# ekinakyurek/Long-Term-Recurrent-Convolutional-NN

Measured on AMD Instinct MI355X. Metric: training images/sec (VGG16+LSTM, COCO, batch 256) at 1/2/4/8 MI355X, higher is better.
Workload: dtype bf16

## Files before the change

long-term-recurrent-convolutional-nn_amd/_lib.py:

```python
import ctypes as C
import os
import subprocess

HERE = os.path.dirname(os.path.abspath(__file__))
CSRC = os.path.join(HERE, "csrc")
LIB_PATH = os.environ.get("LRCN_HIP_LIB") or os.path.join(CSRC, "liblrcn_hip.so")
HEADER = os.path.normpath(os.path.join(HERE, "..", "include", "lrcn.h"))
SAMPLE_HEADER = os.path.normpath(os.path.join(HERE, "..", "include", "lrcn_sample.h"))
SCORE_HEADER = os.path.normpath(os.path.join(HERE, "..", "include", "lrcn_score.h"))
NUCLEUS_HEADER = os.path.normpath(os.path.join(HERE, "..", "include", "lrcn_nucleus.h"))
NBEST_HEADER = os.path.normpath(os.path.join(HERE, "..", "include", "lrcn_nbest.h"))
DIVERSE_HEADER = os.path.normpath(os.path.join(HERE, "..", "include", "lrcn_diverse.h"))
ACTIVITY_HEADER = os.path.normpath(os.path.join(HERE, "..", "include", "lrcn_activity.h"))
ACT_DROPOUT_HEADER = os.path.normpath(os.path.join(HERE, "..", "include", "lrcn_act_dropout.h"))
VARLEN_HEADER = os.path.normpath(os.path.join(HERE, "..", "include", "lrcn_varlen.h"))
CLIP_HEADER = os.path.normpath(os.path.join(HERE, "..", "include", "lrcn_clip.h"))
WEIGHTED_HEADER = os.path.normpath(os.path.join(HERE, "..", "include", "lrcn_weighted.h"))
SCHED_HEADER = os.path.normpath(os.path.join(HERE, "..", "include", "lrcn_sched.h"))
GEMM_DEBUG_HEADER = os.path.normpath(os.path.join(HERE, "..", "include", "lrcn_gemm_debug.h"))
CONV_DEBUG_HEADER = os.path.normpath(os.path.join(HERE, "..", "include", "lrcn_conv_debug.h"))

LRCN_F32, LRCN_BF16, LRCN_FP8 = 0, 1, 2
LRCN_ABI_VERSION = 5
LRCN_OPT_FUSED_UPDATE, LRCN_OPT_DETERMINISTIC, LRCN_OPT_CONV_CHUNK_BYTES = 1, 2, 3
SEGMENTS = ("update", "rec_fwd", "rec_bwd", "embed_gather", "embed_grad", "preprocess", "upload")
EOS, BOS, UNK = 0, 1, 2
CNNOUT = 4096
MAX_T = 28


class LrcnError(RuntimeError):
    pass


class Config(C.Structure):
    _fields_ = [("device", C.c_int), ("E", C.c_int), ("H1", C.c_int), ("H2", C.c_int), ("V", C.c_int),
                ("max_B", C.c_int), ("max_T", C.c_int), ("lstm_dtype", C.c_int), ("vgg_dtype", C.c_int),
                ("max_images", C.c_int), ("n_layers", C.c_int)]


class ActConfig(C.Structure):
    _fields_ = [("device", C.c_int), ("F", C.c_int), ("H", C.c_int), ("C", C.c_int), ("max_B", C.c_int), ("max_T", C.c_int),
                ("dtype", C.c_int), ("deterministic", C.c_int)]


class ActDropout(C.Structure):
    _fields_ = [("p_in", C.c_float), ("p_out", C.c_float), ("seed", C.c_uint64), ("mask_in", C.c_void_p), ("mask_out", C.c_void_p)]


class GemmDebug(C.Structure):
    _fields_ = [("dtype", C.c_int), ("A", C.c_void_p), ("B", C.c_void_p), ("C", C.c_void_p), ("bias", C.c_void_p),
                ("lda", C.c_int64), ("ldb", C.c_int64), ("ldc", C.c_int64), ("M", C.c_int), ("N", C.c_int), ("K", C.c_int),
                ("c_f32", C.c_int), ("beta", C.c_int), ("relu", C.c_int), ("c_is_zero", C.c_int), ("deterministic", C.c_int),
                ("free_cus", C.c_int), ("bg_cus", C.c_int), ("wg_cap", C.c_int)]


class ConvGemmDebug(C.Structure):
    _fields_ = [("dtype", C.c_int), ("x", C.c_void_p), ("w", C.c_void_p), ("bias", C.c_void_p), ("y", C.c_void_p), ("ldc", C.c_int64),
                ("N", C.c_int), ("H", C.c_int), ("W", C.c_int), ("Cin", C.c_int), ("Cout", C.c_int), ("relu", C.c_int), ("pool", C.c_int),
                ("wg_cap", C.c_int)]


class Dropout(C.Structure):
    _fields_ = [("pdrop", C.c_float), ("seed", C.c_uint64), ("mask1", C.c_void_p), ("mask2", C.c_void_p)]


class Sched(C.Structure):
    _fields_ = [("eps", C.c_float), ("temperature", C.c_float), ("seed", C.c_uint64), ("row0", C.c_int64)]


P9 = C.c_void_p * 9
P4 = C.c_void_p * 4
P13 = C.c_void_p * 13

SIGNATURES = {
    "lrcn_create": (C.c_int, [C.POINTER(Config), C.POINTER(C.c_void_p)]),
    "lrcn_destroy": (None, [C.c_void_p]),
# ... 163 lines not shown
CLIP_SIGNATURES = {
    "lrcn_grad_sumsq": (C.c_int, [C.c_void_p, C.c_void_p, C.c_int64, C.c_int, C.c_void_p]),
    "lrcn_grad_sumsq_model": (C.c_int, [C.c_void_p, P9, C.c_int, C.c_void_p]),
    "lrcn_clip_slots": (C.c_int, [C.c_void_p, C.POINTER(C.c_void_p)]),
    "lrcn_clip_set": (C.c_int, [C.c_void_p, C.c_int, C.c_float, C.c_void_p]),
    "lrcn_adam_update_clipped": (C.c_int, [C.c_void_p, P9, P9, P9, P9, C.c_int, C.c_float, C.c_float, C.c_float, C.c_float]),
    "lrcn_adam_update_group_clipped": (C.c_int, [C.c_void_p, P9, P9, P9, P9, C.c_int, C.c_int, C.c_float, C.c_float, C.c_float, C.c_float,
                                                 C.c_void_p]),
    "lrcn_adam_update_flat_clipped": (C.c_int, [C.c_void_p, C.c_void_p, C.c_void_p, C.c_void_p, C.c_void_p, C.c_int64, C.c_int, C.c_float,
                                                C.c_float, C.c_float, C.c_float, C.c_void_p]),
    "lrcn_train_step_clip": (C.c_int, [C.c_void_p, P9, P9, P9, P9, C.c_void_p, C.c_void_p, C.c_int, C.c_int, C.c_int, C.POINTER(Dropout),
                                       C.c_int, C.c_float, C.c_float, C.c_float, C.c_float, C.c_float, C.POINTER(C.c_double)]),
    "lrcn_train_step_var_clip": (C.c_int, [C.c_void_p, P9, P9, P9, P9, C.c_void_p, C.c_void_p, C.POINTER(C.c_int32), C.c_int, C.c_int,
                                           C.c_int64, C.POINTER(Dropout), C.c_int, C.c_float, C.c_float, C.c_float, C.c_float, C.c_float,
                                           C.POINTER(C.c_double)]),
    "lrcn_clip_stats": (C.c_int, [C.c_void_p, C.POINTER(ClipStats)]),
}

GEMM_DEBUG_SIGNATURES = {
    "lrcn_debug_gemm": (C.c_int, [C.c_void_p, C.POINTER(GemmDebug)]),
    "lrcn_debug_conv_gemm": (C.c_int, [C.c_void_p, C.POINTER(ConvGemmDebug)]),
}

CONV_DEBUG_SIGNATURES = {
    "lrcn_debug_conv11": (C.c_int, [C.c_void_p, C.c_void_p, C.c_int, C.c_int, C.c_int, C.POINTER(C.c_float), C.c_void_p, C.c_void_p, C.c_void_p]),
    "lrcn_debug_fp8_cast": (C.c_int, [C.c_void_p, C.c_int, C.c_void_p, C.c_int64, C.c_float, C.c_void_p]),
    "lrcn_debug_amax": (C.c_int, [C.c_void_p, C.c_void_p, C.c_int64, C.c_void_p]),
    "lrcn_debug_conv64_f8": (C.c_int, [C.c_void_p, C.c_void_p, C.c_int, C.c_int, C.c_int, C.c_void_p, C.c_void_p, C.c_int, C.c_float, C.c_void_p]),
    "lrcn_debug_fp8_scales": (C.c_int, [C.c_void_p, C.POINTER(C.c_float)]),
}


def build(force=False):
    srcs = [os.path.join(CSRC, f) for f in os.listdir(CSRC) if f.endswith((".hip", ".h"))] + [HEADER, SAMPLE_HEADER, NUCLEUS_HEADER, SCORE_HEADER, NBEST_HEADER, DIVERSE_HEADER,
                                                                                                   ACTIVITY_HEADER, ACT_DROPOUT_HEADER, VARLEN_HEADER, CLIP_HEADER, WEIGHTED_HEADER, SCHED_HEADER, GEMM_DEBUG_HEADER, CONV_DEBUG_HEADER]
    stale = force or not os.path.exists(LIB_PATH) or os.path.getmtime(LIB_PATH) < max(os.path.getmtime(s) for s in srcs)
    if stale:
        subprocess.check_call(["make", "-s", "-j4", "-C", CSRC, "-f", os.path.join(CSRC, "Makefile")])
    return LIB_PATH


_LIB = None


def lib():
    global _LIB
    if _LIB is None:
        if not os.path.exists(LIB_PATH):
            raise LrcnError("%s is missing: run `python -c 'import __graft_entry__ as g; g.build()'` "
                            "(there is no CPU fallback)" % LIB_PATH)
        import torch
        L = C.CDLL(LIB_PATH)
        for name, (res, args) in list(SIGNATURES.items()) + list(SAMPLE_SIGNATURES.items()) + list(NUCLEUS_SIGNATURES.items()) + list(SCORE_SIGNATURES.items()) + list(NBEST_SIGNATURES.items()) + list(DIVERSE_SIGNATURES.items()) + \
                list(ACTIVITY_SIGNATURES.items()) + list(ACT_DROPOUT_SIGNATURES.items()) + list(VARLEN_SIGNATURES.items()) + list(CLIP_SIGNATURES.items()) + list(WEIGHTED_SIGNATURES.items()) + list(SCHED_SIGNATURES.items()) + \
                list(GEMM_DEBUG_SIGNATURES.items()) + list(CONV_DEBUG_SIGNATURES.items()):
            fn = getattr(L, name)
            fn.restype = res
            fn.argtypes = args
        if L.lrcn_abi_version() != LRCN_ABI_VERSION:
            raise LrcnError("%s implements ABI revision %d, this binding was written against %d (lrcn_config's layout differs)"
                            % (LIB_PATH, L.lrcn_abi_version(), LRCN_ABI_VERSION))
        _LIB = L
    return _LIB


def check(ctx_handle, rc):
    if rc != 0:
        msg = lib().lrcn_last_error(ctx_handle)
        raise LrcnError("liblrcn_hip error %d: %s" % (rc, msg.decode() if msg else "?"))
```

long-term-recurrent-convolutional-nn_amd/csrc/ctx.h:

```cpp
#pragma once
#include <utility>

#include "comm.h"
#include "host.h"
#include "../../include/lrcn_sched.h"

namespace lrcn_impl {

struct VggLayer {
    void *w = nullptr;
    void *w_fused = nullptr;
    float *b = nullptr;
    int Cin = 0, Cout = 0, S = 0, pool = 0;
    void *w8 = nullptr;
    float *sw = nullptr, *escale = nullptr, *ebias = nullptr;
};
constexpr int kFp8First = 3;

}

struct lrcn_ctx {
    lrcn_config cfg{};
    hipStream_t stream = nullptr;
    std::string err;
// ... 80 lines not shown
    int vgg_wg_cap = 0;
    bool vgg_loaded = false;
    bool vgg_fp8 = false, fp8_ready = false;
    float *amax_dev = nullptr;
    float act_scale[13] = {};
    lrcn_impl::VggLayer conv[13];
    void *fc6w = nullptr, *fc7w = nullptr;
    float *fc6b = nullptr, *fc7b = nullptr;
    void *actA = nullptr, *actB = nullptr, *im2col = nullptr, *f6 = nullptr, *img16 = nullptr;
    float *featsRM = nullptr;
    bool prof = false;
    std::vector<std::pair<hipEvent_t, hipEvent_t>> prof_ev;
    size_t prof_used = 0;
    double prof_ms = 0.0;
    int64_t prof_launches = 0;
    int prof_level = 0;
    struct SegProf {
        std::vector<std::pair<hipEvent_t, hipEvent_t>> ev;
        size_t used = 0;
        double ms = 0.0, bytes = 0.0;
        int64_t n = 0;
    } seg[LRCN_SEG_COUNT];
    std::string vgg_routes;
    float *avg_img = nullptr;
    bool avg_on = false;
    void *img_meta = nullptr;
    int img_meta_cap = 0;
    float *pre_f32 = nullptr;
    hipStream_t wg_stream = nullptr;
    bool wg_stream_owned = true;
    hipEvent_t wg_fork[4] = {}, wg_done = nullptr;
    hipEvent_t xc_fork = nullptr, xc_done = nullptr;
    void *wg_ws = nullptr;
    void *pin = nullptr;
    size_t pin_bytes = 0;
    unsigned long long *stamps = nullptr;
    int64_t stamps_n = 0;
    int *tile_ctr = nullptr;
    static constexpr int kStage = 3;
    hipStream_t copy_stream = nullptr;
    uint8_t *stage[kStage] = {};
    hipEvent_t up_done[kStage] = {}, rd_done[kStage] = {};
    bool stage_full[kStage] = {};
    bool stage_read[kStage] = {};
    int stage_next = 0;
    LrcnComm *comm = nullptr;
// ... 18 lines not shown
        auto &sp = c->seg[seg];
        if (sp.used == sp.ev.size()) {
            std::pair<hipEvent_t, hipEvent_t> e;
            if (hipEventCreate(&e.first) != hipSuccess || hipEventCreate(&e.second) != hipSuccess) return;
            sp.ev.push_back(e);
        }
        ev = &sp.ev[sp.used++];
        sp.bytes += bytes;
        sp.n += 1;
        (void)hipEventRecord(ev->first, st);
    }
    ~SegScope() {
        if (ev) (void)hipEventRecord(ev->second, st);
    }
};

inline hipStream_t stream_or_ctx(lrcn_ctx *c, void *stream) { return stream ? reinterpret_cast<hipStream_t>(stream) : c->stream; }
inline void ctx_sizes(const lrcn_ctx *c, int64_t sz[9]) { lrcn_param_sizes_n(c->nl, c->E, c->H1, c->H2, c->V, sz); }
constexpr int kGradGroup[LRCN_GRAD_GROUPS][2] = {{7, 8}, {2, 3}, {4, 5}, {0, 1}, {6, 6}};

int gemm(lrcn_ctx *c, int dtype, const void *A, int64_t lda, const void *B, int64_t ldb, void *C, int64_t ldc, int M, int N, int K,
         const float *bias, bool c_f32, bool beta = false, bool relu = false, bool c_is_zero = false, bool on_wg_stream = false);

#define GEMM(...)                     \
    do {                              \
        int _r = gemm(__VA_ARGS__);   \
        if (_r) return _r;            \
    } while (0)

void set_create_error(const char *msg);
int step_internal(lrcn_ctx *c, const float *const p[9], int B, const DropSpec &d2, bool h_ready = false);
struct LossCall {
    const float *const *p = nullptr;
    const float *feats = nullptr;
    const int32_t *tokens = nullptr;
    int T = 0, B = 0, norm_B = 1;
    int64_t norm_tokens = 0;
    const lrcn_dropout *drop = nullptr;
    float *const *grads = nullptr;
    const int32_t *lens = nullptr;
    const float *row_w = nullptr;
    const lrcn_sched *ss = nullptr;
    int32_t *fed_out = nullptr;
    float *logits_out = nullptr;
    enum Form { PLAIN, VAR, WEIGHTED, SCHED } form = PLAIN;
};
// ... 20 lines not shown
```

long-term-recurrent-convolutional-nn_amd/csrc/gemm.h:

```cpp
#pragma once
#include <hip/hip_runtime.h>
#include <stdint.h>

enum { GEMM_A_PLAIN = 0, GEMM_A_CONV3 = 1 };
enum { GEMM_OUT_PLAIN = 0, GEMM_OUT_CONV = 1, GEMM_OUT_POOL = 2, GEMM_OUT_LSTM_FWD = 3, GEMM_OUT_LSTM_BWD = 4, GEMM_OUT_SMAX_TOPK = 5,
       GEMM_OUT_SMAX_GUMBEL = 6, GEMM_OUT_SMAX_PICK = 7 };

enum { SMAX_KC = 6, SMAX_REC = 16 };
enum { SMAX_MAX_NREC = 256 };
struct SmaxEpi {
    float *part;
    int nrec;
    float temp;
    uint32_t key0, key1;
    int current, S;
    const int32_t *tgt;
};

struct LstmEpi {
    int H;
    int64_t ld_a, ld_h;
    const float *Gx;
    const float *c_prev;
    const int *c_prev_idx;
// ... 46 lines not shown
};

constexpr int kBgMinRows = 256, kBgMaxRows = 512;
inline bool bg_row_window(int rows) { return rows >= kBgMinRows && rows <= kBgMaxRows; }

hipError_t launch_gemm(hipStream_t stream, const GemmArgs &g);
hipError_t launch_gemm_nt(hipStream_t stream, const GemmArgs &g);

void gemm_debug_note_route(const char *route, int cfg);
const char *gemm_debug_last_route();

bool gemm_glds_eligible(const GemmArgs &g);
hipError_t launch_gemm_glds(hipStream_t stream, const GemmArgs &g);
int64_t gemm_glds_blocks(const GemmArgs &g);

int gemm_8p_config(const GemmArgs &g, int64_t *blocks);
int gemm_8p_splitk(const GemmArgs &g, int64_t *blocks);
hipError_t launch_gemm_8p(hipStream_t stream, const GemmArgs &g, int splitk = 1);
hipError_t launch_splitk_reduce(hipStream_t stream, const GemmArgs &g, int splits);

bool gemm_skinny_eligible(const GemmArgs &g);
hipError_t launch_gemm_skinny(hipStream_t stream, const GemmArgs &g);

bool conv64_eligible(int dtype, int Cin, int Cout, int H, int W);
hipError_t launch_conv64(hipStream_t stream, const void *in, const void *w, const float *bias, void *out, int N, int H, int W, int Cout,
                         int relu, int pool, const void *zero_page, float f8_inv_scale = 0.0f, int wg_cap = 0, unsigned long long *stamps = nullptr);
hipError_t launch_conv64_fused11(hipStream_t stream, const void *img16, const void *w11, const float *b11, const void *w,
                                 const float *bias, void *out, int N, int S, const void *zero_page, int wg_cap = 0, unsigned long long *stamps = nullptr);
hipError_t launch_conv64f(hipStream_t stream, const void *img16, const void *w11, const void *w, const float *bias, void *out, int N, int S,
                          const void *zero_page, int wg_cap = 0, unsigned long long *stamps = nullptr);
```

long-term-recurrent-convolutional-nn_amd/csrc/lrcn_api.hip:

```cpp
#include <algorithm>
#include <cmath>

#include "ctx.h"

static thread_local std::string g_create_err;
using namespace lrcn_impl;

constexpr int kBgWgsPerFreeCu = 4;

int lrcn_impl::gemm(lrcn_ctx *c, int dtype, const void *A, int64_t lda, const void *B, int64_t ldb, void *C, int64_t ldc, int M, int N,
         int K, const float *bias, bool c_f32, bool beta, bool relu, bool c_is_zero, bool on_wg_stream) {
    GemmArgs g{};
    g.dtype = dtype;
    g.A = A;
    g.lda = lda;
    g.B = B;
    g.ldb = ldb;
    g.C = C;
    g.ldc = ldc;
    g.M = M;
    g.N = N;
    g.K = gemm_k(dtype, lda, ldb, K);
    g.bias = bias;
    g.c_f32 = c_f32;
    g.beta = beta;
    g.c_is_zero = c_is_zero;
    g.relu = relu;
    g.a_mode = GEMM_A_PLAIN;
    g.out_mode = GEMM_OUT_PLAIN;
    g.zero_page = c->zero_page;
    g.deterministic = c->opt_det;
    g.ws = on_wg_stream ? c->wg_ws : c->gemm_ws;
    g.ws_bytes = c->gemm_ws_bytes;
    if (!lstm_alone(c)) {
        const int free_cus = std::max(c->ncu - c->vgg_wg_cap, 0);
        if (c->cur_B < kBgMinRows) {
            g.free_cus = free_cus;
        } else {
            g.bg_cus = free_cus;
            if (free_cus >= 8) g.wg_cap = free_cus * kBgWgsPerFreeCu;
        }
    }
    hipError_t e = launch_gemm(on_wg_stream ? c->wg_stream : c->stream, g);
    if (e != hipSuccess) FAIL(c, LRCN_EHIP, "gemm M=%d N=%d K=%d: %s", M, N, K, hipGetErrorString(e));
    if (knob_char("LRCN_TRACE_ROUTES") == '1') {
        fprintf(stderr, "gemm M=%d N=%d K=%d %s-> %s\n", M, N, K, on_wg_stream ? "(wg stream) " : "", gemm_debug_last_route());
    }
    return LRCN_OK;
}

void lrcn_impl::set_create_error(const char *msg) { g_create_err = msg; }

int lrcn_impl::step_internal(lrcn_ctx *c, const float *const p[9], int B, const DropSpec &d2, bool h_ready) {
    const int dt = c->dt, E = c->E, H1 = c->H1, H2 = c->H2, h = c->h, V = c->V, X1 = c->X1;
    hipStream_t st = c->stream;
    const bool two = c->nl == 2;
    if (!two) k_concat_x2(st, dt, c->st_x, c->ldX1, c->xcnn, c->ldh, 1, B, E, h, d2);
    if (!h_ready) k_cast_rows(st, dt, c->st_f32[0], H1, B, H1, c->st_h1, c->ldH1);
    GEMM(c, dt, c->st_x, c->ldX1, c->W1x, c->ldX1, c->st_g, 4 * H1, B, 4 * H1, X1, p[1], true);
    GEMM(c, dt, c->st_h1, c->ldH1, c->W1h, c->ldH1, c->st_g, 4 * H1, B, 4 * H1, H1, nullptr, true, true);
    k_lstm_fwd(st, dt, c->st_g, 4 * H1, c->st_f32[1], B, H1, c->st_a, c->ld4H1, c->st_f32[1], c->st_h1, c->ldH1, c->st_f32[0]);
    if (!two) {
        GEMM(c, dt, c->st_h1, c->ldH1, c->Wod, c->ldH2, c->st_logits, c->ldV, B, V, H2, p[8], true);
// ... 370 lines not shown
        k_mul_f32(st, x_lstm, mask1, (int64_t)B * E, c->st_io);
        xsrc = c->st_io;
    }
    k_transpose(st, dt, 1, xsrc, B, E, B, c->st_x, c->ldX1, 0);
    r = step_internal(c, p, B, d2);
    if (r) return r;
    for (int i = 0; i < ns; ++i) k_transpose_f32(st, c->st_f32[i], Hs[i], B, Hs[i], state[i], B);
    k_transpose_f32(st, c->st_logits, c->ldV, B, V, logits, B);
    KCHK(c, "lrcn_step");
    return LRCN_OK;
}

int lrcn_debug_stamps(lrcn_ctx *c, unsigned long long *host_out, int64_t n) {
    DeviceGuard dg(c);
    if (!c || !host_out || n < 1) return LRCN_EINVAL;
    if (!c->stamps || n > c->stamps_n) FAIL(c, LRCN_ESTATE, "no stamps recorded (LRCN_STAMPS=1 and lrcn_bench_conv first), or n > %lld", (long long)c->stamps_n);
    HIPCHK(c, hipStreamSynchronize(c->stream));
    HIPCHK(c, hipMemcpy(host_out, c->stamps, sizeof(unsigned long long) * (size_t)n, hipMemcpyDeviceToHost));
    return LRCN_OK;
}

const char *lrcn_debug_route(lrcn_ctx *c, int which) {
    if (which == 1) return c ? c->vgg_routes.c_str() : "";
    return gemm_debug_last_route();
}

int lrcn_profile(lrcn_ctx *c, int enable) {
    DeviceGuard dg(c);
    if (!c) return LRCN_EINVAL;
    c->prof = enable != 0;
    c->prof_level = enable;
    c->prof_used = 0;
    c->prof_ms = 0.0;
    c->prof_launches = 0;
    for (auto &sp : c->seg) {
        sp.used = 0;
        sp.ms = sp.bytes = 0.0;
        sp.n = 0;
    }
    return LRCN_OK;
}

int lrcn_profile_segment(lrcn_ctx *c, int segment, double *ms, int64_t *brackets, double *bytes) {
    DeviceGuard dg(c);
    if (!c || !ms || !brackets || !bytes || segment < 0 || segment >= LRCN_SEG_COUNT) return LRCN_EINVAL;
    HIPCHK(c, hipDeviceSynchronize());
// ... 31 lines not shown
```

long-term-recurrent-convolutional-nn_amd/csrc/train.hip:

```cpp
#include <cmath>
#include <cstring>

#include "ctx.h"
#include "../../include/lrcn_varlen.h"
#include "../../include/lrcn_clip.h"
#include "../../include/lrcn_weighted.h"
#include "../../include/lrcn_sched.h"

using namespace lrcn_impl;

namespace {

DropSpec make_drop(const lrcn_dropout *d, int which) {
    DropSpec s{};
    s.which = which;
    if (d) {
        s.p = d->pdrop;
        s.seed = d->seed;
        s.mask = which == 1 ? d->mask1 : d->mask2;
        if (s.mask) s.p = 0.0f;
    }
    return s;
}

// ... 277 lines not shown
    if (c->opt_det && !c->logp_rows) DALLOC(c, c->logp_rows, sizeof(double) * (size_t)c->maxS * c->maxB);
    void *const dlog = bwd ? c->dLog : nullptr;
    double *const rows = c->opt_det ? c->logp_rows : nullptr;
    if (q.row_w) k_softmax_xent_weighted(st, dt, c->Logits, c->ldV, c->tok_tgt, M, V, scale, c->logp, dlog, c->ldV, rows, c->roww_dev, B);
    else (q.lens ? k_softmax_xent_masked : k_softmax_xent)(st, dt, c->Logits, c->ldV, c->tok_tgt, M, V, scale, c->logp, dlog, c->ldV, rows);
    c->last_norm = q.norm_B;
    c->last_S = S;
    c->last_tokens = q.lens ? q.norm_tokens : 0;
    KCHK(c, "forward");
    if (!bwd) return LRCN_OK;

    const int64_t ldM = ld64(M), ldB = ld64(B);
    hipStream_t sw = par ? c->wg_stream : st;
    int nfork = 0;
    auto fork = [&]() -> int {
        if (!par) return LRCN_OK;
        HIPCHK(c, hipEventRecord(c->wg_fork[nfork], st));
        HIPCHK(c, hipStreamWaitEvent(sw, c->wg_fork[nfork], 0));
        ++nfork;
        return LRCN_OK;
    };
    auto weight_grad = [&](const void *dY, int64_t ldY, int NY, const void *x, int64_t ldx, int X, const void *Hprev, int64_t ldHp, int Hp,
                           float *dW, float *db) -> int {
        TrPlan pl{};
        auto tr = [&](const void *src, int64_t ld_src, int R, int C, void *dst, int shift) {
            TrDesc &d = pl.d[pl.n++];
            d.src = src; d.ld_src = ld_src; d.R = R; d.C = C; d.dst = dst; d.ld_dst = ldM; d.shift = shift;
        };
        tr(dY, ldY, M, NY, c->TA, 0);
        tr(x, ldx, M, X, c->TB, 0);
        if (Hprev) tr(Hprev, ldHp, M - B, Hp, boff(c->TB, (int64_t)X * ldM, es), M > B ? B : 0);
        k_transpose_multi(sw, dt, pl);
        const int Xh = X + (Hprev ? Hp : 0);
        GEMM(c, dt, c->TA, ldM, c->TB, ldM, dW, Xh, NY, Xh, M, nullptr, true, false, false, false, par);
        if (db) k_colsum(sw, dt, dY, ldY, M, NY, db, c->opt_det);
        return LRCN_OK;
    };
    auto image_embedding_grad = [&]() -> int {
        k_transpose(sw, dt, 1, c->dxcnn, c->ldh, B, h, c->dxcT, ldB, 0);
        k_cast_rows(sw, dt, q.feats, B, LRCN_CNNOUT, B, c->FT, ldB);
        GEMM(c, dt, c->dxcT, ldB, c->FT, ldB, q.grads[5], LRCN_CNNOUT, h, LRCN_CNNOUT, B, nullptr, true, false, false, false, par);
        HIPCHK(c, hipEventRecord(c->grad_ev[2], sw));
        return LRCN_OK;
    };
    auto backward = [&]() -> int {
        if (int e = fork()) return e;
        if (int e = weight_grad(c->dLog, c->ldV, V, Htop, c->ldH2, H2, nullptr, 0, 0, q.grads[7], q.grads[8])) return e;
        HIPCHK(c, hipEventRecord(c->grad_ev[0], sw));
        GEMM(c, dt, c->dLog, c->ldV, c->WoT, c->ldV, two ? c->dH2all : c->dH1all, H2, M, H2, V, nullptr, true);
        if (two) {
            if (int e = lstm_layer_bwd(c, S, B, H2, c->ld4H2, c->A2, c->C2, c->dH2all, c->W2hT, c->dZ2)) return e;
            if (int e = fork()) return e;
            if (int e = weight_grad(c->dZ2, c->ld4H2, 4 * H2, c->X2, c->ldH2, H2, c->H2all, c->ldH2, H2, q.grads[2], q.grads[3])) return e;
        }
        HIPCHK(c, hipEventRecord(c->grad_ev[1], sw));
        if (two) {
            GEMM(c, dt, c->dZ2, c->ld4H2, c->W2xT, c->ld4H2, c->dX2, c->ldH2, M, H2, 4 * H2, nullptr, false);
// ... 256 lines not shown
```

long-term-recurrent-convolutional-nn_amd/csrc/vgg.hip:

```cpp
#include <algorithm>
#include <cstring>

#include "ctx.h"
#include "../../include/lrcn_conv_debug.h"
#include "../../include/lrcn_gemm_debug.h"

using namespace lrcn_impl;

static const int kVggCout[13] = {64, 64, 128, 128, 256, 256, 256, 512, 512, 512, 512, 512, 512};
static const int kVggPool[13] = {0, 1, 0, 1, 0, 0, 1, 0, 0, 1, 0, 0, 1};

namespace {
int stamps_reserve(lrcn_ctx *c, int64_t need) {
    if (need > c->stamps_n) {
        c->stamps = nullptr;
        DALLOC(c, c->stamps, sizeof(unsigned long long) * (size_t)need);
        c->stamps_n = need;
    }
    return LRCN_OK;
}
bool conv64_enabled() { return !knob_off("LRCN_CONV64"); }
constexpr int kTileCtrStride = 8 + 2 * 512;
hipError_t launch_conv_chunked(hipStream_t st, const GemmArgs &g0, int N, int es, int64_t limit_bytes = 0) {
    const int64_t per_img = (int64_t)g0.H * g0.W * g0.Cin * es;
    int64_t cap = ((limit_bytes > 0 ? limit_bytes : 0xF0000000ll) - (limit_bytes > 0 ? 0 : (int64_t)(g0.W + 1) * g0.Cin * es)) / per_img;
    if (limit_bytes > 0 && cap < 1) cap = 1;
    if (N <= cap || cap < 1) return launch_gemm(st, g0);
    const int nch = (int)((N + cap - 1) / cap), per = (N + nch - 1) / nch;
// ... 385 lines not shown
    g.N = d->N;
    g.K = d->K;
    g.bias = d->bias;
    g.c_f32 = d->c_f32 != 0;
    g.beta = d->beta != 0;
    g.c_is_zero = d->c_is_zero != 0;
    g.relu = d->relu != 0;
    g.a_mode = GEMM_A_PLAIN;
    g.out_mode = GEMM_OUT_PLAIN;
    g.zero_page = c->zero_page;
    g.deterministic = d->deterministic != 0;
    g.ws = c->gemm_ws;
    g.ws_bytes = c->gemm_ws_bytes;
    g.free_cus = d->free_cus;
    g.bg_cus = d->bg_cus;
    g.wg_cap = d->wg_cap;
    const hipError_t e = launch_gemm(c->stream, g);
    if (e != hipSuccess)
        FAIL(c, e == hipErrorInvalidValue ? LRCN_EINVAL : LRCN_EHIP, "debug_gemm M=%d N=%d K=%d: %s", d->M, d->N, d->K, hipGetErrorString(e));
    HIPCHK(c, hipStreamSynchronize(c->stream));
    return LRCN_OK;
}

int lrcn_debug_conv_gemm(lrcn_ctx *c, const lrcn_conv_gemm_debug *d) {
    DeviceGuard dg(c);
    if (!c || !d) return LRCN_EINVAL;
    if (d->dtype != LRCN_F32 && d->dtype != LRCN_BF16) FAIL(c, LRCN_EINVAL, "debug_conv_gemm: dtype %d is neither f32 nor bf16", d->dtype);
    if (d->N < 1 || d->H < 2 || d->W < 2 || d->Cin < 1 || d->Cout < 1 || d->ldc < d->Cout || (int64_t)d->N * d->H * d->W > 0x7FFFFFFF ||
        (int64_t)9 * d->Cin > 0x7FFFFFFF)
        FAIL(c, LRCN_EINVAL, "debug_conv_gemm: N=%d H=%d W=%d Cin=%d Cout=%d ldc=%lld", d->N, d->H, d->W, d->Cin, d->Cout, (long long)d->ldc);
    GemmArgs g{};
    g.dtype = d->dtype == LRCN_BF16 ? GEMM_T_BF16 : GEMM_T_F32;
    g.A = d->x;
    g.B = d->w;
    g.ldb = 9 * (int64_t)d->Cin;
    g.C = d->y;
    g.ldc = d->ldc;
    g.M = d->N * d->H * d->W;
    g.N = d->Cout;
    g.K = 9 * d->Cin;
    g.bias = d->bias;
    g.relu = d->relu != 0;
    g.a_mode = GEMM_A_CONV3;
    g.out_mode = d->pool ? GEMM_OUT_POOL : GEMM_OUT_CONV;
    g.H = d->H;
    g.W = d->W;
// ... 452 lines not shown
```

long-term-recurrent-convolutional-nn_amd/lrcn.py:

```python
import ctypes as C

import numpy as np
import torch

from . import _lib
from ._lib import BOS, CNNOUT, EOS, LRCN_BF16, LRCN_F32, LRCN_FP8, UNK, LrcnError

PARAM_NAMES = ("W1", "b1", "W2", "b2", "Wproj", "Wcnn", "Wembed", "Wout", "bout")
VGG_COUT = (64, 64, 128, 128, 256, 256, 256, 512, 512, 512, 512, 512, 512)
VGG_MEAN = (123.68, 116.779, 103.939)


def jl_empty(*dims, device="cuda", dtype=torch.float32):
    t = torch.empty(tuple(reversed(dims)), device=device, dtype=dtype)
    return t.permute(*reversed(range(len(dims))))


def jl_zeros(*dims, device="cuda", dtype=torch.float32):
    t = jl_empty(*dims, device=device, dtype=dtype)
    t.zero_()
    return t


def to_jl(a, device="cuda"):
# ... 787 lines not shown

def debug_route(ctx, which=0):
    r = _lib.lib().lrcn_debug_route(ctx._h, int(which))
    return r.decode() if r else ""


def debug_gemm(ctx, dtype, A, B, Cmat, M, N, K, lda, ldb, ldc, bias=None, c_f32=False, beta=False, relu=False, c_is_zero=False,
               deterministic=False, free_cus=0, bg_cus=0, wg_cap=0):
    def addr(t):
        if t is None:
            return None
        if torch.is_tensor(t):
            if not t.is_cuda:
                raise LrcnError("expected a CUDA (HIP) tensor")
            return C.c_void_p(t.data_ptr())
        return C.c_void_p(int(t))
    g = _lib.GemmDebug(int(dtype), addr(A), addr(B), addr(Cmat), addr(bias), int(lda), int(ldb), int(ldc), int(M), int(N), int(K),
                       int(bool(c_f32)), int(bool(beta)), int(bool(relu)), int(bool(c_is_zero)), int(bool(deterministic)),
                       int(free_cus), int(bg_cus), int(wg_cap))
    ctx._call("lrcn_debug_gemm", C.byref(g))
    return debug_route(ctx, 0)


def debug_conv_gemm(ctx, dtype, x, w, y, N, H, W, Cin, Cout, ldc, bias=None, relu=False, pool=False, wg_cap=0):
    def addr(t):
        if t is None:
            return None
        if torch.is_tensor(t):
            if not t.is_cuda:
                raise LrcnError("expected a CUDA (HIP) tensor")
            return C.c_void_p(t.data_ptr())
        return C.c_void_p(int(t))
    g = _lib.ConvGemmDebug(int(dtype), addr(x), addr(w), addr(bias), addr(y), int(ldc), int(N), int(H), int(W), int(Cin), int(Cout),
                           int(bool(relu)), int(bool(pool)), int(wg_cap))
    ctx._call("lrcn_debug_conv_gemm", C.byref(g))
    return debug_route(ctx, 0)


def synthetic_vgg_weights(seed=1, device="cuda", bias_std=0.0):
    g = torch.Generator(device=device)
    g.manual_seed(seed)
    conv_w, conv_b = [], []
    cin = 3
    for cout in VGG_COUT:
        w = jl_empty(3, 3, cin, cout, device=device)
        w.copy_(torch.randn((3, 3, cin, cout), generator=g, device=device) * float(np.sqrt(2.0 / (9 * cin))))
# ... 11 lines not shown
```

Before: 37640.

## Add transposed-input bf16 GEMM kernel for LSTM weight gradients, skipping explicit transposes

Adds a dedicated MFMA GEMM kernel that computes dY^T·[x,Hprev] directly from row-major inputs. It uses transposing LDS reads (ds_read_b64_tr_b16), a 4-stage async global-to-LDS pipeline, and two segments per launch. The LSTM weight-gradient path uses it by default for bf16, which removes the transpose kernels and the scratch buffers they wrote. It adds a large hand-tuned kernel with tile heuristics. If the kernel is ineligible, the old transpose-plus-GEMM path still runs.

```diff
diff --git a/include/lrcn_gemm_tn_debug.h b/include/lrcn_gemm_tn_debug.h
--- /dev/null
+++ b/include/lrcn_gemm_tn_debug.h
@@ -0,0 +1,28 @@
+#ifndef LRCN_GEMM_TN_DEBUG_H
+#define LRCN_GEMM_TN_DEBUG_H
+
+#include "lrcn.h"
+
+#ifdef __cplusplus
+extern "C" {
+#endif
+
+typedef struct lrcn_gemm_tn_debug {
+    const void *A;
+    const void *B;
+    float *C;
+    int64_t lda, ldb, ldc;
+    int M, NA, NB;
+    int shift;
+    int tile;
+} lrcn_gemm_tn_debug;
+
+int lrcn_debug_gemm_tn(lrcn_ctx *ctx, const lrcn_gemm_tn_debug *g);
+
+int lrcn_debug_set_wgrad_tn(lrcn_ctx *ctx, int on);
+
+#ifdef __cplusplus
+}
+#endif
+
+#endif
diff --git a/long-term-recurrent-convolutional-nn_amd/_lib.py b/long-term-recurrent-convolutional-nn_amd/_lib.py
--- a/long-term-recurrent-convolutional-nn_amd/_lib.py
+++ b/long-term-recurrent-convolutional-nn_amd/_lib.py
@@ -18,6 +18,7 @@
 WEIGHTED_HEADER = os.path.normpath(os.path.join(HERE, "..", "include", "lrcn_weighted.h"))
 SCHED_HEADER = os.path.normpath(os.path.join(HERE, "..", "include", "lrcn_sched.h"))
 GEMM_DEBUG_HEADER = os.path.normpath(os.path.join(HERE, "..", "include", "lrcn_gemm_debug.h"))
+GEMM_TN_DEBUG_HEADER = os.path.normpath(os.path.join(HERE, "..", "include", "lrcn_gemm_tn_debug.h"))
 CONV_DEBUG_HEADER = os.path.normpath(os.path.join(HERE, "..", "include", "lrcn_conv_debug.h"))
 
 LRCN_F32, LRCN_BF16, LRCN_FP8 = 0, 1, 2
@@ -53,6 +54,11 @@
                 ("lda", C.c_int64), ("ldb", C.c_int64), ("ldc", C.c_int64), ("M", C.c_int), ("N", C.c_int), ("K", C.c_int),
                 ("c_f32", C.c_int), ("beta", C.c_int), ("relu", C.c_int), ("c_is_zero", C.c_int), ("deterministic", C.c_int),
                 ("free_cus", C.c_int), ("bg_cus", C.c_int), ("wg_cap", C.c_int)]
+
+
+class GemmTnDebug(C.Structure):
+    _fields_ = [("A", C.c_void_p), ("B", C.c_void_p), ("C", C.c_void_p), ("lda", C.c_int64), ("ldb", C.c_int64), ("ldc", C.c_int64),
+                ("M", C.c_int), ("NA", C.c_int), ("NB", C.c_int), ("shift", C.c_int), ("tile", C.c_int)]
 
 
 class ConvGemmDebug(C.Structure):
@@ -262,6 +268,11 @@
     "lrcn_debug_conv_gemm": (C.c_int, [C.c_void_p, C.POINTER(ConvGemmDebug)]),
 }
 
+GEMM_TN_DEBUG_SIGNATURES = {
+    "lrcn_debug_gemm_tn": (C.c_int, [C.c_void_p, C.POINTER(GemmTnDebug)]),
+    "lrcn_debug_set_wgrad_tn": (C.c_int, [C.c_void_p, C.c_int]),
+}
+
 CONV_DEBUG_SIGNATURES = {
     "lrcn_debug_conv11": (C.c_int, [C.c_void_p, C.c_void_p, C.c_int, C.c_int, C.c_int, C.POINTER(C.c_float), C.c_void_p, C.c_void_p, C.c_void_p]),
     "lrcn_debug_fp8_cast": (C.c_int, [C.c_void_p, C.c_int, C.c_void_p, C.c_int64, C.c_float, C.c_void_p]),
@@ -273,7 +284,7 @@
 
 def build(force=False):
     srcs = [os.path.join(CSRC, f) for f in os.listdir(CSRC) if f.endswith((".hip", ".h"))] + [HEADER, SAMPLE_HEADER, NUCLEUS_HEADER, SCORE_HEADER, NBEST_HEADER, DIVERSE_HEADER,
-                                                                                                   ACTIVITY_HEADER, ACT_DROPOUT_HEADER, VARLEN_HEADER, CLIP_HEADER, WEIGHTED_HEADER, SCHED_HEADER, GEMM_DEBUG_HEADER, CONV_DEBUG_HEADER]
+                                                                                                   ACTIVITY_HEADER, ACT_DROPOUT_HEADER, VARLEN_HEADER, CLIP_HEADER, WEIGHTED_HEADER, SCHED_HEADER, GEMM_DEBUG_HEADER, GEMM_TN_DEBUG_HEADER, CONV_DEBUG_HEADER]
     stale = force or not os.path.exists(LIB_PATH) or os.path.getmtime(LIB_PATH) < max(os.path.getmtime(s) for s in srcs)
     if stale:
         subprocess.check_call(["make", "-s", "-j4", "-C", CSRC, "-f", os.path.join(CSRC, "Makefile")])
@@ -293,7 +304,7 @@
         L = C.CDLL(LIB_PATH)
         for name, (res, args) in list(SIGNATURES.items()) + list(SAMPLE_SIGNATURES.items()) + list(NUCLEUS_SIGNATURES.items()) + list(SCORE_SIGNATURES.items()) + list(NBEST_SIGNATURES.items()) + list(DIVERSE_SIGNATURES.items()) + \
                 list(ACTIVITY_SIGNATURES.items()) + list(ACT_DROPOUT_SIGNATURES.items()) + list(VARLEN_SIGNATURES.items()) + list(CLIP_SIGNATURES.items()) + list(WEIGHTED_SIGNATURES.items()) + list(SCHED_SIGNATURES.items()) + \
-                list(GEMM_DEBUG_SIGNATURES.items()) + list(CONV_DEBUG_SIGNATURES.items()):
+                list(GEMM_DEBUG_SIGNATURES.items()) + list(GEMM_TN_DEBUG_SIGNATURES.items()) + list(CONV_DEBUG_SIGNATURES.items()):
             fn = getattr(L, name)
             fn.restype = res
             fn.argtypes = args
diff --git a/long-term-recurrent-convolutional-nn_amd/csrc/ctx.h b/long-term-recurrent-convolutional-nn_amd/csrc/ctx.h
--- a/long-term-recurrent-convolutional-nn_amd/csrc/ctx.h
+++ b/long-term-recurrent-convolutional-nn_amd/csrc/ctx.h
@@ -126,6 +126,8 @@
         int64_t n = 0;
     } seg[LRCN_SEG_COUNT];
     std::string vgg_routes;
+    bool wgrad_tn = true;
+    std::string wgrad_route;
     float *avg_img = nullptr;
     bool avg_on = false;
     void *img_meta = nullptr;
@@ -190,6 +192,8 @@
 int gemm(lrcn_ctx *c, int dtype, const void *A, int64_t lda, const void *B, int64_t ldb, void *C, int64_t ldc, int M, int N, int K,
          const float *bias, bool c_f32, bool beta = false, bool relu = false, bool c_is_zero = false, bool on_wg_stream = false);
 
+int bg_wg_cap(const lrcn_ctx *c);
+
 #define GEMM(...)                     \
     do {                              \
         int _r = gemm(__VA_ARGS__);   \
diff --git a/long-term-recurrent-convolutional-nn_amd/csrc/gemm.h b/long-term-recurrent-convolutional-nn_amd/csrc/gemm.h
--- a/long-term-recurrent-convolutional-nn_amd/csrc/gemm.h
+++ b/long-term-recurrent-convolutional-nn_amd/csrc/gemm.h
@@ -92,6 +92,31 @@
 bool gemm_skinny_eligible(const GemmArgs &g);
 hipError_t launch_gemm_skinny(hipStream_t stream, const GemmArgs &g);
 
+struct GemmTnSeg {
+    const void *A;
+    int64_t lda;
+    const void *B;
+    int64_t ldb;
+    float *C;
+    int64_t ldc;
+    int M;
+    int NB;
+    int tile0, vec;
+};
+struct GemmTnArgs {
+    int dtype;
+    GemmTnSeg seg[2];
+    int nseg;
+    int M;
+    int NA;
+    int wg_cap;
+    int tile;
+    const void *zero_page;
+    int tiles;
+};
+bool gemm_tn_eligible(const GemmTnArgs &g);
+hipError_t launch_gemm_tn(hipStream_t stream, const GemmTnArgs &g);
+
 bool conv64_eligible(int dtype, int Cin, int Cout, int H, int W);
 hipError_t launch_conv64(hipStream_t stream, const void *in, const void *w, const float *bias, void *out, int N, int H, int W, int Cout,
                          int relu, int pool, const void *zero_page, float f8_inv_scale = 0.0f, int wg_cap = 0, unsigned long long *stamps = nullptr);
diff --git a/long-term-recurrent-convolutional-nn_amd/csrc/gemm_tn.hip b/long-term-recurrent-convolutional-nn_amd/csrc/gemm_tn.hip
--- /dev/null
+++ b/long-term-recurrent-convolutional-nn_amd/csrc/gemm_tn.hip
@@ -0,0 +1,219 @@
+#include <type_traits>
+#include <utility>
+
+#include "common.h"
+#include "gemm.h"
+
+namespace {
+
+typedef __attribute__((address_space(3))) void lds_void;
+typedef const __attribute__((address_space(1))) void glb_void;
+typedef unsigned u32x2 __attribute__((ext_vector_type(2)));
+typedef unsigned u32x4 __attribute__((ext_vector_type(4)));
+
+constexpr int TN_IMG_COLS = 128;
+constexpr int TN_BK = 32;
+constexpr int TN_NBUF = 4;
+constexpr int TN_IPT = 4;
+constexpr int TN_IMG_BYTES = TN_BK * TN_IMG_COLS * 2;
+static_assert((TN_NBUF - 2) * TN_IPT <= 48, "vmcnt is a 6-bit counter");
+
+template <int NWA, int NWB, int FA, int FB> struct TnCfg {
+    static constexpr int TA = NWA * FA * 16, TB = NWB * FB * 16, NW = NWA * NWB, THREADS = NW * 64;
+    static constexpr int NIA = TA / TN_IMG_COLS, NIB = TB / TN_IMG_COLS;
+    static constexpr int STAGE_BYTES = (NIA + NIB) * TN_IMG_BYTES, LDS_BYTES = TN_NBUF * STAGE_BYTES;
+    static_assert(TA % TN_IMG_COLS == 0 && TB % TN_IMG_COLS == 0 && 2 * (NIA + NIB) == NW, "two waves stage one image");
+};
+
+template <int... I, typename F> __device__ __forceinline__ void tn_static_for(std::integer_sequence<int, I...>, F &&f) {
+    (f(std::integral_constant<int, I>{}), ...);
+}
+
+__device__ __forceinline__ int tn_swz(int k) { return ((k & 3) << 2) | ((k >> 2) & 3); }
+__device__ __forceinline__ int tn_off(int k, int ch) { return 256 * k + 16 * (ch ^ tn_swz(k)); }
+
+template <int N> __device__ __forceinline__ void tn_wait_vmcnt() { asm volatile("s_waitcnt vmcnt(%0)" ::"n"(N) : "memory"); }
+template <int N> __device__ __forceinline__ void tn_wait_lgkmcnt() {
+    asm volatile("s_waitcnt lgkmcnt(%0)" ::"n"(N) : "memory");
+    __builtin_amdgcn_sched_barrier(0);
+}
+__device__ __forceinline__ u32x2 tn_read_tr(unsigned addr) {
+    u32x2 r;
+    asm volatile("ds_read_b64_tr_b16 %0, %1" : "=v"(r) : "v"(addr) : "memory");
+    return r;
+}
+__device__ __forceinline__ bf16x8 tn_pack(u32x2 lo, u32x2 hi) { return __builtin_bit_cast(bf16x8, u32x4{lo[0], lo[1], hi[0], hi[1]}); }
+
+template <int NWA, int NWB, int FA, int FB>
+__global__ __launch_bounds__(NWA * NWB * 64) void gemm_tn_kernel(const GemmTnArgs g) {
+    using Cfg = TnCfg<NWA, NWB, FA, FB>;
+    constexpr int TA = Cfg::TA, TB = Cfg::TB, NIA = Cfg::NIA, STAGE_BYTES = Cfg::STAGE_BYTES;
+    extern __shared__ __attribute__((aligned(16))) unsigned char tn_lds[];
+    const int tid = threadIdx.x, lane = tid & 63;
+    const int wave = __builtin_amdgcn_readfirstlane(tid >> 6);
+    const int wa = wave / NWB, wb = wave % NWB;
+    const int grp = lane >> 4, li = lane & 15, q = li >> 2, p = li & 3;
+    const unsigned lds0 = (unsigned)(uintptr_t)(__attribute__((address_space(3))) unsigned char *)tn_lds;
+    unsigned addr_a[FA][2], addr_b[FB][2];
+#pragma unroll
+    for (int r = 0; r < 2; ++r) {
+        const int k = 8 * grp + 4 * r + q;
+#pragma unroll
+        for (int j = 0; j < FA; ++j) {
+            const int col = (wa * FA + j) * 16;
+            addr_a[j][r] = lds0 + (col / TN_IMG_COLS) * TN_IMG_BYTES + tn_off(k, (col % TN_IMG_COLS) / 8 + (p >> 1)) + 8 * (p & 1);
+        }
+#pragma unroll
+        for (int j = 0; j < FB; ++j) {
+            const int col = (wb * FB + j) * 16;
+            addr_b[j][r] = lds0 + (NIA + col / TN_IMG_COLS) * TN_IMG_BYTES + tn_off(k, (col % TN_IMG_COLS) / 8 + (p >> 1)) + 8 * (p & 1);
+        }
+    }
+    const int img = wave >> 1;
+    const bool stage_a = img < NIA;
+    const int img_col = (stage_a ? img : img - NIA) * TN_IMG_COLS;
+    const int pc0 = (wave & 1) * 4;
+    const unsigned char *zp = static_cast<const unsigned char *>(g.zero_page) + li * 16;
+
+    for (int tile = blockIdx.x; tile < g.tiles; tile += gridDim.x) {
+        const GemmTnSeg s = g.seg[(g.nseg > 1 && tile >= g.seg[1].tile0) ? 1 : 0];
+        const int tb_n = (s.NB + TB - 1) / TB;
+        const int t = tile - s.tile0, a0 = (t / tb_n) * TA, b0 = (t % tb_n) * TB;
+        const int M = s.M, nk = (M + TN_BK - 1) / TN_BK;
+        const bf16_t *P = static_cast<const bf16_t *>(stage_a ? s.A : s.B);
+        const int ld = (int)(stage_a ? s.lda : s.ldb), ncols = stage_a ? g.NA : s.NB, c0 = (stage_a ? a0 : b0) + img_col;
+        int src_off[TN_IPT], src_row[TN_IPT];
+#pragma unroll
+        for (int i = 0; i < TN_IPT; ++i) {
+            const int row = 4 * (pc0 + i) + grp, col = c0 + 8 * (li ^ tn_swz(row));
+            src_row[i] = row;
+            src_off[i] = col < ncols ? row * ld + col : -1;
+        }
+        auto stage = [&](int kt, int slot, bool live) {
+            unsigned char *dst = tn_lds + slot * STAGE_BYTES + img * TN_IMG_BYTES + pc0 * 1024;
+#pragma unroll
+            for (int i = 0; i < TN_IPT; ++i) {
+                const bool ok = live && src_off[i] >= 0 && kt * TN_BK + src_row[i] < M;
+                const void *src = ok ? static_cast<const void *>(P + ((int64_t)kt * TN_BK * ld + src_off[i])) : static_cast<const void *>(zp);
+                __builtin_amdgcn_global_load_lds((glb_void *)src, (lds_void *)(dst + i * 1024), 16, 0, 0);
+            }
+        };
+
+        f32x4 acc[FB][FA];
+#pragma unroll
+        for (int jb = 0; jb < FB; ++jb)
+#pragma unroll
+            for (int ja = 0; ja < FA; ++ja) acc[jb][ja] = f32x4{0.f, 0.f, 0.f, 0.f};
+
+#pragma unroll
+        for (int t0 = 0; t0 < TN_NBUF - 1; ++t0) stage(t0, t0, t0 < nk);
+        for (int kt = 0; kt < nk; ++kt) {
+            tn_wait_vmcnt<(TN_NBUF - 2) * TN_IPT>();
+            __builtin_amdgcn_s_barrier();
+            const int nxt = kt + TN_NBUF - 1;
+            stage(nxt, nxt % TN_NBUF, nxt < nk);
+            const unsigned cur = (unsigned)(kt % TN_NBUF) * STAGE_BYTES;
+            u32x2 rb[FB][2], ra[FA][2];
+#pragma unroll
+            for (int j = 0; j < FB; ++j) {
+                rb[j][0] = tn_read_tr(addr_b[j][0] + cur);
+                rb[j][1] = tn_read_tr(addr_b[j][1] + cur);
+            }
+#pragma unroll
+            for (int j = 0; j < FA; ++j) {
+                ra[j][0] = tn_read_tr(addr_a[j][0] + cur);
+                ra[j][1] = tn_read_tr(addr_a[j][1] + cur);
+            }
+            tn_static_for(std::make_integer_sequence<int, FA>{}, [&](auto col) {
+                constexpr int ja = decltype(col)::value;
+                tn_wait_lgkmcnt<2 * (FA - 1 - ja)>();
+#pragma unroll
+                for (int jb = 0; jb < FB; ++jb)
+                    acc[jb][ja] = __builtin_amdgcn_mfma_f32_16x16x32_bf16(tn_pack(rb[jb][0], rb[jb][1]), tn_pack(ra[ja][0], ra[ja][1]), acc[jb][ja], 0, 0, 0);
+            });
+            __builtin_amdgcn_sched_barrier(0);
+        }
+        tn_wait_vmcnt<0>();
+
+        float *C = s.C;
+#pragma unroll
+        for (int ja = 0; ja < FA; ++ja) {
+            const int row = a0 + 16 * (FA * wa + ja) + li;
+            if (row >= g.NA) continue;
+            float *crow = C + (int64_t)row * s.ldc;
+#pragma unroll
+            for (int jb = 0; jb < FB; ++jb) {
+                const int col = b0 + 16 * (FB * wb + jb) + 4 * grp;
+                const f32x4 v = acc[jb][ja];
+                if (col + 4 <= s.NB && s.vec == 4) {
+                    *reinterpret_cast<f32x4 *>(crow + col) = v;
+                } else if (col + 4 <= s.NB && s.vec == 2) {
+                    *reinterpret_cast<float2 *>(crow + col) = make_float2(v[0], v[1]);
+                    *reinterpret_cast<float2 *>(crow + col + 2) = make_float2(v[2], v[3]);
+                } else {
+#pragma unroll
+                    for (int e = 0; e < 4; ++e)
+                        if (col + e < s.NB) crow[col + e] = v[e];
+                }
+            }
+        }
+        tn_wait_vmcnt<0>();
+        __syncthreads();
+    }
+}
+
+bool seg_ok(const GemmTnSeg &s, int NA, int M) {
+    if (!s.A || !s.B || !s.C || s.M < 0 || s.M > M || s.NB < 1) return false;
+    if (((uintptr_t)s.A & 15) || ((uintptr_t)s.B & 15) || ((uintptr_t)s.C & 3)) return false;
+    if ((s.lda & 7) || (s.ldb & 7) || s.lda < NA || s.ldb < s.NB || s.ldc < s.NB) return false;
+    const int64_t rows = (int64_t)s.M + TN_BK;
+    if (rows * s.lda >= (1ll << 31) || rows * s.ldb >= (1ll << 31) || (int64_t)NA * s.ldc >= (1ll << 31)) return false;
+    return true;
+}
+
+}
+
+bool gemm_tn_eligible(const GemmTnArgs &g) {
+    if (g.dtype != GEMM_T_BF16 || g.M < 1 || g.NA < 1 || g.nseg < 1 || g.nseg > 2) return false;
+    if (g.tile != 0 && g.tile != 128 && g.tile != 256) return false;
+    if (!g.zero_page || ((uintptr_t)g.zero_page & 15)) return false;
+    for (int k = 0; k < g.nseg; ++k)
+        if (!seg_ok(g.seg[k], g.NA, g.M)) return false;
+    int64_t tiles = 0;
+    for (int k = 0; k < g.nseg; ++k) tiles += (int64_t)cdiv(g.NA, 128) * cdiv(g.seg[k].NB, 128);
+    return tiles <= 0x7FFFFFFF;
+}
+
+template <int NWA, int NWB, int FA, int FB> static hipError_t launch_tn_cfg(hipStream_t stream, GemmTnArgs &g) {
+    using Cfg = TnCfg<NWA, NWB, FA, FB>;
+    int tiles = 0;
+    for (int k = 0; k < g.nseg; ++k) {
+        g.seg[k].tile0 = tiles;
+        tiles += cdiv(g.NA, Cfg::TA) * cdiv(g.seg[k].NB, Cfg::TB);
+    }
+    g.tiles = tiles;
+    const int blocks = g.wg_cap > 0 && g.wg_cap < tiles ? g.wg_cap : tiles;
+    static LdsAttrMask lds_set{0};
+    if (hipError_t e = set_max_lds(reinterpret_cast<const void *>(gemm_tn_kernel<NWA, NWB, FA, FB>), Cfg::LDS_BYTES, lds_set)) return e;
+    hipLaunchKernelGGL((gemm_tn_kernel<NWA, NWB, FA, FB>), dim3(blocks), dim3(Cfg::THREADS), Cfg::LDS_BYTES, stream, g);
+    return hipGetLastError();
+}
+
+constexpr int kTnBigMinTiles = 64;
+
+hipError_t launch_gemm_tn(hipStream_t stream, const GemmTnArgs &g0) {
+    if (!gemm_tn_eligible(g0)) {
+        gemm_debug_note_route("?", -1);
+        return hipErrorInvalidValue;
+    }
+    GemmTnArgs g = g0;
+    int64_t big_tiles = 0;
+    for (int k = 0; k < g.nseg; ++k) {
+        GemmTnSeg &s = g.seg[k];
+        big_tiles += (int64_t)cdiv(g.NA, 256) * cdiv(s.NB, 256);
+        s.vec = (((uintptr_t)s.C & 15) == 0 && s.ldc % 4 == 0) ? 4 : (((uintptr_t)s.C & 7) == 0 && s.ldc % 2 == 0) ? 2 : 1;
+    }
+    const bool big = g.tile == 256 || (g.tile != 128 && big_tiles >= kTnBigMinTiles);
+    gemm_debug_note_route("tn", -1);
+    return big ? launch_tn_cfg<2, 4, 8, 4>(stream, g) : launch_tn_cfg<2, 2, 4, 4>(stream, g);
+}
diff --git a/long-term-recurrent-convolutional-nn_amd/csrc/lrcn_api.hip b/long-term-recurrent-convolutional-nn_amd/csrc/lrcn_api.hip
--- a/long-term-recurrent-convolutional-nn_amd/csrc/lrcn_api.hip
+++ b/long-term-recurrent-convolutional-nn_amd/csrc/lrcn_api.hip
@@ -7,6 +7,12 @@
 using namespace lrcn_impl;
 
 constexpr int kBgWgsPerFreeCu = 4;
+
+int lrcn_impl::bg_wg_cap(const lrcn_ctx *c) {
+    if (lstm_alone(c) || c->cur_B < kBgMinRows) return 0;
+    const int free_cus = std::max(c->ncu - c->vgg_wg_cap, 0);
+    return free_cus >= 8 ? free_cus * kBgWgsPerFreeCu : 0;
+}
 
 int lrcn_impl::gemm(lrcn_ctx *c, int dtype, const void *A, int64_t lda, const void *B, int64_t ldb, void *C, int64_t ldc, int M, int N,
          int K, const float *bias, bool c_f32, bool beta, bool relu, bool c_is_zero, bool on_wg_stream) {
@@ -38,7 +44,7 @@
             g.free_cus = free_cus;
         } else {
             g.bg_cus = free_cus;
-            if (free_cus >= 8) g.wg_cap = free_cus * kBgWgsPerFreeCu;
+            g.wg_cap = bg_wg_cap(c);
         }
     }
     hipError_t e = launch_gemm(on_wg_stream ? c->wg_stream : c->stream, g);
@@ -455,6 +461,7 @@
 
 const char *lrcn_debug_route(lrcn_ctx *c, int which) {
     if (which == 1) return c ? c->vgg_routes.c_str() : "";
+    if (which == 2) return c ? c->wgrad_route.c_str() : "";
     return gemm_debug_last_route();
 }
 
diff --git a/long-term-recurrent-convolutional-nn_amd/csrc/train.hip b/long-term-recurrent-convolutional-nn_amd/csrc/train.hip
--- a/long-term-recurrent-convolutional-nn_amd/csrc/train.hip
+++ b/long-term-recurrent-convolutional-nn_amd/csrc/train.hip
@@ -323,6 +323,27 @@
     };
     auto weight_grad = [&](const void *dY, int64_t ldY, int NY, const void *x, int64_t ldx, int X, const void *Hprev, int64_t ldHp, int Hp,
                            float *dW, float *db) -> int {
+        const int Xh = X + (Hprev ? Hp : 0);
+        if (dt == GEMM_T_BF16 && c->wgrad_tn) {
+            GemmTnArgs t{};
+            t.dtype = dt;
+            t.M = M;
+            t.NA = NY;
+            t.nseg = Hprev ? 2 : 1;
+            t.wg_cap = bg_wg_cap(c);
+            t.zero_page = c->zero_page;
+            t.seg[0] = GemmTnSeg{dY, ldY, x, ldx, dW, Xh, M, X, 0, 0};
+            if (Hprev) t.seg[1] = GemmTnSeg{boff(dY, (int64_t)B * ldY, es), ldY, Hprev, ldHp, dW + X, Xh, M - B, Hp, 0, 0};
+            if (gemm_tn_eligible(t)) {
+                const hipError_t e = launch_gemm_tn(sw, t);
+                if (e != hipSuccess) FAIL(c, LRCN_EHIP, "gemm_tn M=%d NA=%d NB=%d: %s", M, NY, Xh, hipGetErrorString(e));
+                if (knob_char("LRCN_TRACE_ROUTES") == '1')
+                    fprintf(stderr, "gemm_tn M=%d NA=%d NB=%d+%d %s-> %s\n", M, NY, X, Xh - X, par ? "(wg stream) " : "", gemm_debug_last_route());
+                c->wgrad_route = gemm_debug_last_route();
+                if (db) k_colsum(sw, dt, dY, ldY, M, NY, db, c->opt_det);
+                return LRCN_OK;
+            }
+        }
         TrPlan pl{};
         auto tr = [&](const void *src, int64_t ld_src, int R, int C, void *dst, int shift) {
             TrDesc &d = pl.d[pl.n++];
@@ -332,8 +353,8 @@
         tr(x, ldx, M, X, c->TB, 0);
         if (Hprev) tr(Hprev, ldHp, M - B, Hp, boff(c->TB, (int64_t)X * ldM, es), M > B ? B : 0);
         k_transpose_multi(sw, dt, pl);
-        const int Xh = X + (Hprev ? Hp : 0);
         GEMM(c, dt, c->TA, ldM, c->TB, ldM, dW, Xh, NY, Xh, M, nullptr, true, false, false, false, par);
+        c->wgrad_route = gemm_debug_last_route();
         if (db) k_colsum(sw, dt, dY, ldY, M, NY, db, c->opt_det);
         return LRCN_OK;
     };
diff --git a/long-term-recurrent-convolutional-nn_amd/csrc/vgg.hip b/long-term-recurrent-convolutional-nn_amd/csrc/vgg.hip
--- a/long-term-recurrent-convolutional-nn_amd/csrc/vgg.hip
+++ b/long-term-recurrent-convolutional-nn_amd/csrc/vgg.hip
@@ -4,6 +4,7 @@
 #include "ctx.h"
 #include "../../include/lrcn_conv_debug.h"
 #include "../../include/lrcn_gemm_debug.h"
+#include "../../include/lrcn_gemm_tn_debug.h"
 
 using namespace lrcn_impl;
 
@@ -435,6 +436,39 @@
     return LRCN_OK;
 }
 
+int lrcn_debug_gemm_tn(lrcn_ctx *c, const lrcn_gemm_tn_debug *d) {
+    DeviceGuard dg(c);
+    if (!c || !d) return LRCN_EINVAL;
+    if (d->shift < 0 || d->shift > d->M) FAIL(c, LRCN_EINVAL, "debug_gemm_tn: shift %d outside [0, M = %d]", d->shift, d->M);
+    GemmTnArgs g{};
+    g.dtype = GEMM_T_BF16;
+    g.nseg = 1;
+    g.M = d->M;
+    g.NA = d->NA;
+    g.zero_page = c->zero_page;
+    g.tile = d->tile;
+    g.seg[0].A = d->A ? boff(d->A, (int64_t)d->shift * d->lda, sizeof(bf16_t)) : nullptr;
+    g.seg[0].lda = d->lda;
+    g.seg[0].B = d->B;
+    g.seg[0].ldb = d->ldb;
+    g.seg[0].C = d->C;
+    g.seg[0].ldc = d->ldc;
+    g.seg[0].M = d->M - d->shift;
+    g.seg[0].NB = d->NB;
+    const hipError_t e = launch_gemm_tn(c->stream, g);
+    if (e != hipSuccess)
+        FAIL(c, e == hipErrorInvalidValue ? LRCN_EINVAL : LRCN_EHIP, "debug_gemm_tn M=%d NA=%d NB=%d: %s", d->M, d->NA, d->NB, hipGetErrorString(e));
+    HIPCHK(c, hipStreamSynchronize(c->stream));
+    return LRCN_OK;
+}
+
+int lrcn_debug_set_wgrad_tn(lrcn_ctx *c, int on) {
+    if (!c) return LRCN_EINVAL;
+    if (on != 0 && on != 1) FAIL(c, LRCN_EINVAL, "debug_set_wgrad_tn takes 0 or 1 (got %d)", on);
+    c->wgrad_tn = on != 0;
+    return LRCN_OK;
+}
+
 int lrcn_debug_conv_gemm(lrcn_ctx *c, const lrcn_conv_gemm_debug *d) {
     DeviceGuard dg(c);
     if (!c || !d) return LRCN_EINVAL;
diff --git a/long-term-recurrent-convolutional-nn_amd/lrcn.py b/long-term-recurrent-convolutional-nn_amd/lrcn.py
--- a/long-term-recurrent-convolutional-nn_amd/lrcn.py
+++ b/long-term-recurrent-convolutional-nn_amd/lrcn.py
@@ -833,6 +833,24 @@
     return debug_route(ctx, 0)
 
 
+def debug_gemm_tn(ctx, A, B, Cmat, M, NA, NB, lda, ldb, ldc, shift=0, tile=0):
+    def addr(t):
+        if t is None:
+            return None
+        if torch.is_tensor(t):
+            if not t.is_cuda:
+                raise LrcnError("expected a CUDA (HIP) tensor")
+            return C.c_void_p(t.data_ptr())
+        return C.c_void_p(int(t))
+    g = _lib.GemmTnDebug(addr(A), addr(B), addr(Cmat), int(lda), int(ldb), int(ldc), int(M), int(NA), int(NB), int(shift), int(tile))
+    ctx._call("lrcn_debug_gemm_tn", C.byref(g))
+    return debug_route(ctx, 0)
+
+
+def debug_set_wgrad_tn(ctx, on):
+    ctx._call("lrcn_debug_set_wgrad_tn", int(bool(on)))
+
+
 def debug_conv_gemm(ctx, dtype, x, w, y, N, H, W, Cin, Cout, ldc, bias=None, relu=False, pool=False, wg_cap=0):
     def addr(t):
         if t is None:
```

Result: no change. 37800, median of 6 (+0.4%).
